# ArthurBrussee/brush

Hardware: AMD Instinct MI355X
Metric: train views/sec @ 1M Gaussians, 1080p (fwd + L1/SSIM loss + bwd + Adam per view) (higher is better)
Workload: dtype f32

## Files before the change

### brush_amd/_ffi.py

```python
import ctypes as C
import os

_DIR = os.path.dirname(os.path.abspath(__file__))
LIB_PATH = os.environ.get("BRUSH_HIP_LIB") or os.path.join(_DIR, "libbrush_hip.so")

FLAG_MIP = 1
FLAG_BWD_INFO = 2
FLAG_SMOOTH_CUTOFF = 4
FLAG_SLICED_LISTS = 8

fp = C.POINTER(C.c_float)
u32p = C.POINTER(C.c_uint32)


class BhCamera(C.Structure):
    _fields_ = [
        ("vm", C.c_float * 12),
        ("fx", C.c_float), ("fy", C.c_float), ("cx", C.c_float), ("cy", C.c_float),
        ("lim_pos_x", C.c_float), ("lim_pos_y", C.c_float),
        ("lim_neg_x", C.c_float), ("lim_neg_y", C.c_float),
        ("cam_pos", C.c_float * 3),
        ("img_w", C.c_uint32), ("img_h", C.c_uint32),
        ("tile_row_begin", C.c_uint32), ("tile_row_end", C.c_uint32),
        ("model", C.c_uint32), ("dist", C.c_float * 8), ("half_max_render_fov", C.c_float),
# ... 440 lines not shown

ABI_VERSION = 7
STRUCT_MIRRORS = (BhCamera, BhRenderOut, BhLossConfig, BhTrainConfig, BhTrainState, BhTrainBatch, BhTrainStats, BhRefineConfig, BhRefineStats, BhPlyInfo)

_lib = None
_lib_th = None
TEST_HOOKS_LIB_PATH = os.path.join(_DIR, "libbrush_hip_testhooks.so")
TEST_HOOK_SYMBOLS = {"bh_debug_fill_train_scratch": (C.c_int, [C.c_void_p, C.c_uint32]),
                     "bh_debug_split_counts": (C.c_int, [C.c_void_p, C.POINTER(C.c_uint32)]),
                     "bh_debug_depth_sort": (C.c_int, [C.c_void_p, C.c_void_p, C.c_void_p, C.c_void_p, C.c_uint32, C.c_void_p, C.c_void_p, C.c_void_p, C.c_void_p,
                                                       C.POINTER(C.c_int), C.POINTER(C.c_uint32)]),
                     "bh_debug_depth_deal": (C.c_int, [C.c_void_p, C.c_void_p, C.c_void_p, C.c_void_p, C.c_uint32, C.c_void_p, C.c_void_p, C.c_void_p, C.c_void_p,
                                                       C.c_uint32, C.c_uint32, C.POINTER(C.c_uint64), C.POINTER(C.c_int)]),
                     "bh_debug_dsort_deal_counts": (C.c_int, [C.c_void_p, C.POINTER(C.c_uint32)]),
                     "bh_debug_set_deal_capacity": (C.c_int, [C.c_void_p, C.c_uint32]),
                     "bh_debug_image_loss_window": (C.c_int, [C.c_void_p, C.c_void_p, C.c_void_p, C.c_uint32, C.c_uint32, C.POINTER(BhLossConfig), C.c_float, C.c_uint32,
                                                              C.c_uint32, C.c_void_p, C.c_void_p])}


class BrushHipError(RuntimeError):
    pass


def _bind(path, symbols):
    if not os.path.exists(path):
        raise BrushHipError(
            "%s not found: build it with `python -c 'import __graft_entry__ as g; g.build()'` "
            "(hipcc --offload-arch=gfx950). There is no CPU fallback." % path)
    lib = C.CDLL(path)
    for name, (res, args) in symbols.items():
# ... 25 lines not shown
```

### brush_amd/csrc/api.hip

```cpp
#include <cmath>
#include <cstdlib>
#include <cstdio>
#include <algorithm>
#include <cstring>
#include <new>

#include "../../include/brush_hip_intrinsics.h"
#include "context.h"
#include "depth_deal.h"
#include "device_rng.h"
#include "param_table.h"

namespace bh {

__global__ __launch_bounds__(256) void zero_two_kernel(float4* __restrict__ a, size_t na, float4* __restrict__ b, size_t nb) {
    const size_t stride = (size_t)gridDim.x * 256;
    const float4 z = make_float4(0.0f, 0.0f, 0.0f, 0.0f);
    for (size_t i = (size_t)blockIdx.x * 256 + threadIdx.x; i < na + nb; i += stride) {
        if (i < na) a[i] = z;
        else b[i - na] = z;
    }
}

int set_error(bh_ctx* ctx, int code, const std::string& msg) {
// ... 301 lines not shown
}
bool parse_flag(const char* v, bool* out) {
    uint32_t x = 0;
    if (!parse_u32(v, 0, 1, &x)) return false;
    *out = x != 0;
    return true;
}
struct Option { const char* name; const char* help; bool (*apply)(bh_ctx* c, const char* v); };
const Option kOptions[] = {
    {"cut_min_pairs", "u32: a view whose last frame had fewer pairs keeps complete lists (= bh_set_list_cut_threshold)",
     [](bh_ctx* c, const char* v) { return parse_u32(v, 0, 0xFFFFFFFFu, &c->cut_min_pairs); }},
    {"cut_margin_pct", "0..10000: base margin behind a tile's last useful splat, % of its depth rank (default 150)",
     [](bh_ctx* c, const char* v) { return parse_u32(v, 0, 10000, &c->knob_cut_margin_pct); }},
    {"cut_margin_fixed", "0|1: the margin is cut_margin_pct for every frame instead of adaptive",
     [](bh_ctx* c, const char* v) { return parse_flag(v, &c->knob_fixed_margin); }},
    {"cut_ctrl", "up:down:floor:gap_exp — the margin controller's constants (default 1.5:0.998:0.5:0.3333)", [](bh_ctx* c, const char* v) {
        float a = 0, b = 0, d = 0, e = 0;
        if (sscanf(v, "%f:%f:%f:%f", &a, &b, &d, &e) != 4 || !(a >= 1.0f && b > 0.0f && b <= 1.0f && d > 0.0f && e >= 0.0f && e <= 1.0f)) return false;
        c->ctrl_up = a; c->ctrl_down = b; c->ctrl_floor = d; c->ctrl_gap_exp = e;
        return true;
    }},
    {"cut_sort_all", "0|1: with per-tile cuts, still depth-sort every visible splat",
     [](bh_ctx* c, const char* v) { return parse_flag(v, &c->knob_cut_sort_all); }},
    {"auto_exact_share", "0..1: a view whose last cut frame listed more than this share of its pairs renders complete lists (default 0.9; 0 = never)", [](bh_ctx* c, const char* v) {
        char* end = nullptr;
        const float x = strtof(v, &end);
        if (end == v || *end != '\0' || !(x >= 0.0f && x <= 1.0f)) return false;
        c->auto_exact_share = x;
        return true;
    }},
    {"no_view_hash", "0|1: frames without a view id share ONE table instead of being keyed by their camera",
     [](bh_ctx* c, const char* v) { return parse_flag(v, &c->knob_no_view_hash); }},
    {"k16_order", "0 index order | 1 by the view's last per-tile work | 2 dealt: the forward blend's tile order",
     [](bh_ctx* c, const char* v) { return parse_u32(v, 0, 2, &c->knob_k16_order); }},
// ... 262 lines not shown
    const float* transforms = req.transforms;
    const float* sh_coeffs = req.sh_coeffs;
    const float* raw_opacities = req.raw_opacities;
    ctx->have_forward = false;
    ctx->clears.begin_forward();
    const bool mip = flags & BH_FLAG_MIP;
    Frame f;
    f.bwd_info = flags & BH_FLAG_BWD_INFO; f.smooth = flags & BH_FLAG_SMOOTH_CUTOFF;
    f.bg[0] = req.bg[0]; f.bg[1] = req.bg[1]; f.bg[2] = req.bg[2];
    f.u = make_uniforms(req.cam);
    if (f.u.tile_y0 >= f.u.tile_y1 || f.u.tile_y1 > f.u.tile_bh) return set_error(ctx, BH_ERR_INVALID_ARG, "tile_row window must satisfy begin < end <= ceil(img_h / 16)");
    f.num_tiles = f.u.tile_bw * f.u.tile_bh;
    const size_t npad = n ? n : 1;

    constexpr size_t counter_set_bytes = COUNTER_SET_BYTES, counter_set_words = COUNTER_SET_BYTES / 4, counter_read_bytes = COUNTER_READ_BYTES;
    auto* counter_pairs = (uint32_t*)ensure(ctx, SLOT_COUNTERS, 2 * counter_set_bytes + 64);
    uint32_t* dev_sums = counter_pairs ? counter_pairs + 2 * counter_set_words : nullptr;
    uint32_t* counters = counter_pairs ? counter_pairs + counter_set_words * (ctx->counter_phase & 1u) : nullptr;
    auto* depth_keys = (uint32_t*)ensure(ctx, SLOT_DEPTH_KEYS, npad * 4);
    auto* isect_counts = (uint32_t*)ensure(ctx, SLOT_ISECT_COUNTS, npad * 4);
    auto* max_radius = req.max_radius ? req.max_radius : (float*)ensure(ctx, SLOT_MAX_RADIUS, npad * 4);
    f.proj_by_gid = (float*)ensure(ctx, SLOT_PROJECTED_BY_GID, npad * 9 * 4);
    if (!counters || !depth_keys || !isect_counts || !max_radius || !f.proj_by_gid) return BH_ERR_OOM;

    f.gfc = (uint32_t*)ensure(ctx, SLOT_GLOBAL_FROM_COMPACT, npad * 4);
    auto* depths_sorted = (uint32_t*)ensure(ctx, SLOT_DEPTHS_SORTED, npad * 4);
    if (!f.gfc || !depths_sorted) return BH_ERR_OOM;
    const bool bwd_jobs = f.bwd_info && ctx->knob_bwd_jobs && !ctx->knob_no_lpt && !((flags & BH_FLAG_SLICED_LISTS) && ctx->slice_fraction > 0.0f);
    const size_t lpt_words = LPT_HEADER_WORDS + (size_t)8 * LPT_CLASSES * band_slots(f.num_tiles);
    auto* tile_offsets = (uint32_t*)ensure(ctx, SLOT_TILE_OFFSETS, ((size_t)f.num_tiles * 2 + lpt_words) * 4);
    f.visible = (f.bwd_info && req.visible) ? req.visible : (float*)ensure(ctx, SLOT_VISIBLE, (f.bwd_info ? npad : 1) * 4);
// ... 33 lines not shown
    bool k5_queued = false;
    uint32_t spec_pair_cap = 0;
    float* spec_projected = nullptr;
    float4* spec_vc = nullptr;
    uint32_t *spec_tile_ids = nullptr, *spec_isect_gids = nullptr;
    if (n > 0) {
        fused_scan = depth_sort_supported(n) && !ctx->knob_generic_depth_sort;
        const bool sums_on_device = fused_scan && !ctx->knob_readback_copy;
        bool* spl_written = nullptr;
        uint32_t* spl_listed = nullptr;
        uint32_t* spl = view_splitters(view, cut_active, &spl_written, &spl_listed);
        if (!spl && ctx->dsort_spl) { spl = ctx->dsort_spl; spl_written = &ctx->dsort_spl_written; spl_listed = &ctx->dsort_spl_keys; }
        DealArgs dealt;
        {
            ProfScope ps(ctx, "ProjectSplats");
            if (!ctx->counters_ready) BH_HIP(ctx, hipMemsetAsync(counter_pairs, 0, 2 * counter_set_bytes, ctx->stream));
            ctx->counters_ready = false;
            ForwardPrep prep;
            prep.next_counters = reinterpret_cast<unsigned long long*>(counter_pairs + counter_set_words * ((ctx->counter_phase & 1u) ^ 1u));
            prep.visible = visible_words ? reinterpret_cast<uint32_t*>(f.visible) : nullptr;
            prep.visible_words = (uint32_t)visible_words;
            prep.tile_table = tile_offsets;
            prep.tile_words = f.num_tiles * 2 + LPT_HEADER_WORDS;
            prep.slice_table = slice_tab;
            prep.slice_words = (uint32_t)slice_words;
            prep.list_all_visible = ctx->knob_cut_sort_all;
            if (view && ctx->knob_k16_order && n >= 8u * 256u) {
                const uint32_t win_t = f.u.tile_bw * (f.u.tile_y1 - f.u.tile_y0);
                tile_order = (uint32_t*)ensure(ctx, SLOT_TILE_ORDER, ((size_t)8 * band_slots(win_t) + SPLIT_TAIL_WORDS) * 4);
                if (!tile_order) return BH_ERR_OOM;
                prep.order_work = vtab + (size_t)f.num_tiles;
// ... 48 lines not shown
                spec_projected = (float*)ensure(ctx, SLOT_PROJECTED, npad * 9 * 4);
                spec_vc = f.bwd_info ? (float4*)ensure(ctx, SLOT_V_COMBINED, npad * 10 * 4 + 16) : nullptr;
                if (!spec_projected || (f.bwd_info && !spec_vc)) return BH_ERR_OOM;
                spec_tile_ids = (uint32_t*)ctx->slots[SLOT_TILE_IDS].ptr;
                spec_isect_gids = (uint32_t*)ctx->slots[SLOT_ISECT_GIDS].ptr;
                spec_pair_cap = (uint32_t)std::min<size_t>(cap_pairs, 0xFFFFFFFEull);
                ProfScope ps(ctx, "MapGaussiansToIntersect");
                BH_TRY(launch_map_gaussians(ctx, n, f.u, f.proj_by_gid, f.gfc, spec_projected, cum_early, spec_tile_ids, spec_isect_gids, spec_vc,
                                            spec_vc ? (uint32_t)(((size_t)n * 10 + 3) / 4) : 0u, 0xFFFFFFFFu, cut_active ? slice_tab : nullptr,
                                            cut_active ? vtab : nullptr, cut_active ? depths_sorted : nullptr, dev_sums + (cut_active ? 3 : 0), spec_pair_cap));
                k5_queued = true;
            }
        }
        if (poll_tag) BH_TRY(wait_host_tag(ctx, reinterpret_cast<const volatile uint32_t*>(hslots) + HOST_SUM_WORDS - 1u, ctx->readback_tag, "count readback"));
        else BH_HIP(ctx, hipEventSynchronize(ctx->readback_ev));
        if (ctx->gate_learn) {
            ctx->gate_learn = false;
            ctx->far_direct = reinterpret_cast<const volatile uint32_t*>(ctx->host_counters)[HOST_GATE_WORD] != 0u;
        }
        unsigned long long hc[4] = {0ull, 0ull, 0ull, 0ull};
        if (sums_on_device) {
            const volatile unsigned long long* hs = hslots;
            for (uint32_t c = 0; c < COUNTER_K1_U64; ++c) hc[c] = hs[c];
        } else {
            for (uint32_t k = 0; k < COUNTER_SLOTS; ++k)
                for (uint32_t c = 0; c < COUNTER_K1_U64; ++c) hc[c] += hslots[COUNTER_K1_U64 * k + c];
        }
        if (hc[1] > 0xFFFFFFFFull) return set_error(ctx, BH_ERR_UNSUPPORTED, "more than 2^32-1 tile intersections");
        nv_true = (uint32_t)hc[0];
        f.ni = (uint32_t)hc[1];
// ... 38 lines not shown
    if (bwd_jobs) {
        const uint32_t listed = cut_active ? near_total : f.ni;
        const uint32_t ckpt_cap = (uint32_t)std::min<uint64_t>((uint64_t)listed / BWD_SEG + f.num_tiles + 1u, BWD_CKPT_MAX_SLOTS);
        f.rs.jobs.ckpt = (float4*)ensure(ctx, SLOT_BWD_CKPT, (size_t)ckpt_cap * 256 * sizeof(float4));
        f.rs.jobs.ckpt_cap = ckpt_cap;
        f.rs.jobs.top_cap = band_slots(f.num_tiles) + ckpt_cap;
        f.rs.jobs.top_list = (uint32_t*)ensure(ctx, SLOT_BWD_TOPLIST, (size_t)8 * f.rs.jobs.top_cap * 4);
        if (!f.rs.jobs.ckpt || !f.rs.jobs.top_list) return BH_ERR_OOM;
    }
    if (view) {
        f.rs.zcut = vtab;
        f.rs.depth_keys_sorted = depths_sorted;
        f.rs.nv = f.nv;
        f.rs.cut_active = by_cut;
        f.rs.margin_pct = cut_margin_pct(ctx, view);
        f.rs.work = vtab + (size_t)f.num_tiles;
        f.rs.order = tile_order;
        f.rs.order_mode = ctx->knob_k16_order;
        f.rs.split = tile_split;
#ifdef BH_TEST_HOOKS
        ctx->last_split = tile_split;
#endif
    }
    const uint32_t win_tiles = f.u.tile_bw * (f.u.tile_y1 - f.u.tile_y0);
    const float class_width_raw = (float)f.ni / (float)(win_tiles ? win_tiles : 1u) / 64.0f;
    f.class_width = ctx->knob_lpt_linear ? (class_width_raw < 8.0f ? 8.0f : class_width_raw) : 0.0f;
    f.lpt = (f.bwd_info && !ctx->knob_no_lpt) ? tile_offsets + (size_t)f.num_tiles * 2 : nullptr;
    f.out_f32 = f.bwd_info ? (float*)out_img : nullptr;
    f.out_u8 = f.bwd_info ? nullptr : (uint32_t*)out_img;

// ... 117 lines not shown
    r.intersect_counts = isect_counts;
    r.depths_sorted = (float*)depths_sorted;
    r.tile_offsets_far = sliced ? f.tile_offsets_far : nullptr;
    r.list_budget = f.budget;
    r.generation = ++ctx->generation;
    ctx->clears.stamp(r.generation);
    *out = r;
    ForwardState& latest = ctx->latest;
    latest.out = r;
    latest.uniforms = f.u;
    latest.n = n; latest.sh_degree = sh_degree; latest.flags = flags;
    latest.bg[0] = f.bg[0]; latest.bg[1] = f.bg[1]; latest.bg[2] = f.bg[2];
    latest.lpt = f.lpt;
    latest.jobs = f.rs.jobs;
    ctx->have_forward = true;
    if (view) view_rendered(view, f.ni);
    return 0;
}

extern "C" {

int bh_set_list_slicing(bh_ctx* ctx, float near_share) {
    if (!ctx) return BH_ERR_INVALID_ARG;
    if (near_share != near_share || near_share > 1.0f) return set_error(ctx, BH_ERR_INVALID_ARG, "set_list_slicing: the near slice's share must be <= 1 (<= 0: automatic)");
    ctx->slice_fraction = near_share > 0.0f ? near_share : 0.0f;
    return 0;
}

int bh_set_list_cut_threshold(bh_ctx* ctx, uint32_t min_pairs) {
    if (!ctx) return BH_ERR_INVALID_ARG;
    ctx->cut_min_pairs = min_pairs;
// ... 8 lines not shown

int bh_forget_views(bh_ctx* ctx) {
    if (!ctx) return BH_ERR_INVALID_ARG;
    BH_HIP(ctx, hipSetDevice(ctx->device));
    if (ctx->far_job.pending) BH_TRY(finish_far_slice(ctx, nullptr));
    if (ctx->dsort_spl) { BH_HIP(ctx, hipMemsetAsync(ctx->dsort_spl, 0, DSORT_SPL_STRIDE * 4, ctx->stream)); ctx->dsort_spl_written = false; ctx->dsort_spl_keys = 0u; }
    if (ctx->views.empty()) return 0;
    BH_HIP(ctx, hipStreamSynchronize(ctx->stream));
    deliver_pending_loss(ctx);
    for (auto& kv : ctx->views)
        if (kv.second.zcut) (void)hipFree(kv.second.zcut);
    ctx->views.clear();
    ctx->casual_views = 0;
    for (uint64_t& k : ctx->seen_keys) k = 0ull;
    ctx->far_job.view = nullptr;
    ctx->margin_scale = 1.0f;
    return 0;
}

float bh_last_list_share(bh_ctx* ctx) { return ctx ? ctx->last_slice_share : 0.0f; }
uint32_t bh_far_slices_queued(bh_ctx* ctx) { return ctx ? ctx->far_launches : 0u; }
uint32_t bh_view_table_count(bh_ctx* ctx) { return ctx ? (uint32_t)ctx->views.size() : 0u; }

}

namespace bh {

int backward_impl(bh_ctx* ctx, const ForwardState& fs, const float* v_output, const BackwardCall& call) {
    const float *transforms = call.transforms, *sh_coeffs = call.sh_coeffs, *raw_opacities = call.raw_opacities;
    float *v_transforms = call.v_transforms, *v_sh_coeffs = call.v_sh_coeffs, *v_raw_opacities = call.v_raw_opacities, *v_refine_weight = call.v_refine_weight;
    const size_t span_floats = call.span_floats;
// ... 390 lines not shown
            ctx->deal_fallbacks++;
            rc = depth_sort_scan(ctx, keys, minmax, counts, n, out_keys, out_vals, cum, nullptr, nullptr, nullptr, 0u, nullptr, spl, &written);
            if (rc == 0) rc = check_hip(ctx, hipStreamSynchronize(ctx->stream), "debug_depth_deal: sync");
        }
    } else {
        (void)hipStreamSynchronize(ctx->stream);
    }
    (void)hipFree(d.ctr);
    return rc;
}
extern "C" int bh_debug_set_deal_capacity(bh_ctx* ctx, uint32_t cap) {
    if (!ctx) return BH_ERR_INVALID_ARG;
    ctx->deal_cap_override = cap;
    return 0;
}
extern "C" int bh_debug_dsort_deal_counts(bh_ctx* ctx, uint32_t* out) {
    if (!ctx || !out) return BH_ERR_INVALID_ARG;
    out[0] = ctx->deal_frames;
    out[1] = ctx->deal_fallbacks;
    return 0;
}
extern "C" int bh_debug_image_loss_window(bh_ctx* ctx, const float* img_hwc4, const uint32_t* gt_packed, uint32_t h, uint32_t w, const BhLossConfig* cfg,
                                          float alpha_weight, uint32_t tile_y0, uint32_t tile_y1, float* loss_out, float* v_output) {
    if (!ctx) return BH_ERR_INVALID_ARG;
    if (!img_hwc4 || !gt_packed || !cfg || !loss_out || !v_output || h == 0 || w == 0)
        return set_error(ctx, BH_ERR_INVALID_ARG, "debug_image_loss_window: bad argument");
    if (tile_y0 >= tile_y1) return set_error(ctx, BH_ERR_INVALID_ARG, "debug_image_loss_window: empty tile-row window");
    BH_HIP(ctx, hipSetDevice(ctx->device));
    const size_t hw = (size_t)h * w;
    const bool alpha = alpha_weight > 0.0f;
// ... 7 lines not shown
```

### brush_amd/csrc/context.h

```cpp
#pragma once
#include <hip/hip_runtime.h>
#include <stdint.h>

#include <memory>
#include <string>
#include <unordered_map>
#include <vector>

#include "../../include/brush_hip.h"
#include "../../include/brush_hip_lpips.h"
#include "../../include/brush_hip_image.h"
#include "../../include/brush_hip_exposure.h"
#include "../../include/brush_hip_bilagrid.h"
#include "../../include/brush_hip_depth_loss.h"
#include "../../include/brush_hip_normal_loss.h"
#include "../../include/brush_hip_distortion.h"
#include "../../include/brush_hip_mesh.h"
#include "../../include/brush_hip_features.h"
#include "../../include/brush_hip_feature_train.h"
#include "../../include/brush_hip_envmap.h"
#include "device_math.h"

namespace bh {

enum Slot : int {
    SLOT_COUNTERS = 0,
    SLOT_DEPTH_KEYS,
    SLOT_ISECT_COUNTS,
    SLOT_MAX_RADIUS,
    SLOT_SORT_KEYS_A,
    SLOT_SORT_KEYS_B,
    SLOT_SORT_VALS_A,
    SLOT_SORT_VALS_B,
    SLOT_SORT_HIST,
    SLOT_COMM_SCRATCH,
// ... 72 lines not shown
};

constexpr int MAX_PROF = 32;

constexpr uint32_t COUNTER_SLOTS = 128;
constexpr uint32_t COUNTER_K1_U64 = 4;
constexpr size_t COUNTER_SET_BYTES = COUNTER_SLOTS * 8 * COUNTER_K1_U64 + COUNTER_SLOTS * 8;
constexpr uint32_t COUNTER_SET_U64 = (uint32_t)(COUNTER_SET_BYTES / 8);
constexpr uint32_t COUNTER_MINMAX_WORD = COUNTER_SLOTS * 2 * COUNTER_K1_U64;
constexpr uint32_t SLICE_CTRL_WORDS = 8;
constexpr uint32_t SORT_GROUP_BLOCKS = 32;
constexpr uint32_t FAR_GROUP_BLOCKS = 64;
constexpr size_t COUNTER_READ_BYTES = COUNTER_SLOTS * 8 * COUNTER_K1_U64;
constexpr uint32_t HOST_SUM_WORDS = 2 * COUNTER_K1_U64 + 1;
constexpr uint32_t HOST_DEAL_WORD = HOST_SUM_WORDS;
constexpr size_t HOST_LOSS_WORD = 16 + COUNTER_READ_BYTES / 4;
constexpr size_t HOST_GATE_WORD = HOST_LOSS_WORD + 16;
constexpr size_t HOST_GATE_TAG_WORD = HOST_GATE_WORD + 1;
constexpr size_t HOST_COUNTERS_BYTES = 64 + COUNTER_READ_BYTES + 64 + 64;

struct Profiler {
    int level = 0;
    const char* names[MAX_PROF];
    float ms[MAX_PROF];
    uint32_t calls[MAX_PROF];
    int count = 0;
    struct Pending { int idx; hipEvent_t a, b; };
    std::vector<Pending> pending;
    std::vector<hipEvent_t> pool;
    hipEvent_t ext_a = nullptr, ext_b = nullptr;
};

constexpr uint32_t ZCUT_ALL = 0xFFFFFFFEu;
BH_DEV bool zcut_near(uint32_t key, uint32_t cut) { return (key >> 1) <= (cut >> 1); }
struct ViewState {
    uint32_t* zcut = nullptr;
    uint32_t tile_bw = 0, tile_bh = 0;
    bool seeded = false;
    uint32_t exact_frames = 0;
    uint32_t penalty = 0;
    uint64_t last_used = 0;
    uint32_t gap = 0;
    uint32_t last_pairs = 0;
    uint32_t complete_frames = 0;
    bool spl_written[2] = {false, false};
    uint32_t spl_keys[2] = {0, 0};
    bool casual = false;
};
constexpr uint32_t CUT_MIN_PAIRS = 1500000u;
constexpr uint32_t LPT_CLASSES = 64;
constexpr uint32_t LPT_HEADER_WORDS = 8 * LPT_CLASSES + 64;
constexpr uint32_t BWD_SEG = 128;
constexpr uint32_t BWD_MAX_SEGS = 64;
struct BwdJobs {
    float4* ckpt = nullptr;
    uint32_t ckpt_cap = 0;
    uint32_t* top_list = nullptr;
    uint32_t top_cap = 0;
// ... 38 lines not shown
    uint32_t* done_bits = nullptr;
    uint32_t* unsat_count = nullptr;
    uint32_t* gate_host = nullptr;
    float* state = nullptr;
    const uint32_t* offsets_near = nullptr;
    uint32_t* zcut = nullptr;
    const uint32_t* depth_keys_sorted = nullptr;
    uint32_t nv = 0;
    bool cut_active = false;
    uint32_t* live_bands = nullptr;
    uint32_t* work = nullptr;
    const uint32_t* order = nullptr;
    uint32_t order_mode = 1;
    uint32_t* split = nullptr;
    uint32_t margin_pct = 150;
    BwdJobs jobs{};
};

struct ForwardRequest {
    BhCamera cam{};
    uint32_t n = 0, sh_degree = 0, flags = 0;
    const float* transforms = nullptr;
    const float* sh_coeffs = nullptr;
    const float* raw_opacities = nullptr;
    float bg[3] = {0, 0, 0};
    uint32_t view_id = 0;
    float* visible = nullptr;
    float* max_radius = nullptr;
    size_t visible_floats = 0;
    float* grad_begin = nullptr;
// ... 174 lines not shown
    int comm_rank = 0, comm_world = 1;
    float slice_fraction = 0.0f;
    float last_slice_share = 1.0f;
    bool far_direct = false;
    uint32_t readback_tag = 0;
    uint32_t gate_tag = 0;
    bool gate_signal_queued = false;
    bool gate_learn = false;
    uint32_t far_launches = 0;
    std::unordered_map<uint64_t, bh::ViewState> views;
    uint64_t seen_keys[bh::SEEN_KEYS] = {};
    uint32_t seen_pos = 0;
    uint32_t casual_views = 0;
    uint32_t view_id = 0;
    uint64_t view_clock = 0;
    float margin_scale = 1.0f;
    float ctrl_up = 1.5f, ctrl_down = 0.998f, ctrl_floor = 0.5f, ctrl_gap_exp = 1.0f / 3.0f;
    uint32_t cut_min_pairs = bh::CUT_MIN_PAIRS;
    bool knob_spec_k5 = true;
    bool knob_event_waits = false;
    bool knob_readback_copy = false;
    bool knob_no_view_hash = false;
    bool knob_fixed_margin = false;
    bool knob_cut_sort_all = false;
    uint32_t feature_chunk = 0;
    uint32_t knob_band_mode = 1;
    uint32_t knob_k16_waves = 0;
    uint32_t knob_k16_split = 250;
    uint32_t knob_k16_split_min = bh::SPLIT_MIN_WORK;
    uint32_t knob_k16_split_of_max = 45;
    const uint32_t* last_split = nullptr;
    uint32_t knob_k16_order = 1;
// ... 84 lines not shown
int launch_bilagrid_slice(bh_ctx* ctx, const bh_bilagrid* tab, uint32_t view, const float* img, uint32_t h, uint32_t w, float* out);
int launch_bilagrid_backward(bh_ctx* ctx, bh_bilagrid* tab, uint32_t view, const float* img, const float* v_sliced, uint32_t h, uint32_t w, float* v_img,
                             float tv_weight, bool update);
int launch_bilagrid_tv(bh_ctx* ctx, const bh_bilagrid* tab, uint32_t view, float* value, float weight, float* accum, float* accum_host);
float* bilagrid_tv_scratch(bh_ctx* ctx);
int check_envmap_frame(bh_ctx* ctx, const BhCamera* cam, uint32_t h, uint32_t w, const char* who);
int launch_envmap_composite(bh_ctx* ctx, const bh_envmap* map, const BhCamera& cam, const float* img, uint32_t h, uint32_t w, float* out);
int launch_envmap_backward(bh_ctx* ctx, bh_envmap* map, const BhCamera& cam, const float* img, const float* v_out, uint32_t h, uint32_t w, float* v_img,
                           bool update, float gscale, bool check_host);
int launch_envmap_adam(bh_ctx* ctx, bh_envmap* map, float gscale);
ViewState* frame_view(bh_ctx* ctx, const ForwardRequest& req, uint32_t tile_bw, uint32_t tile_bh, bool casual);
bool cut_this_frame(const bh_ctx* ctx, ViewState* vs, bool allow_cut);
uint32_t* view_table(const ViewState* vs);
uint32_t* view_splitters(ViewState* vs, bool cut, bool** written, uint32_t** listed = nullptr);
uint32_t cut_margin_pct(const bh_ctx* ctx, const ViewState* vs);
uint32_t list_budget(bh_ctx* ctx, ViewState* cut_view, uint32_t near_total, uint32_t ni);
void view_rendered(ViewState* vs, uint32_t ni);
int enqueue_far_slice(bh_ctx* ctx, const FarJob& j);
int finish_far_slice(bh_ctx* ctx, bool* launched);
bool far_job_decides_first(const bh_ctx* ctx);
void drop_far_job(bh_ctx* ctx);
inline void deliver_pending_loss(bh_ctx* ctx) {
    if (ctx->pending_loss_dst) {
        *ctx->pending_loss_dst = reinterpret_cast<const volatile float*>(ctx->host_counters)[HOST_LOSS_WORD];
        ctx->pending_loss_dst = nullptr;
    }
}
int check_hip(bh_ctx* ctx, hipError_t e, const char* what);
int lpips_train_term(bh_ctx* ctx, const float* img_hwc4, const uint32_t* gt_packed, uint32_t h, uint32_t w, const float* bg, float* v_output,
                     float* loss, float* loss_host);
std::string ply_header_comments(uint32_t sh_degree, bool render_mip, const float* up_axis);
enum ResizeOut : int { RESIZE_OUT_U8 = 0, RESIZE_OUT_PACKED = 1, RESIZE_OUT_PACKED_PREMUL = 2 };
// ... 163 lines not shown
```

### brush_amd/csrc/depth_sort.hip

```cpp
#include <cstddef>

#include "context.h"
#include "depth_deal.h"
#include "sort_groups.h"

namespace bh {

constexpr int DS_WG = 256;
constexpr int DS_WAVES = DS_WG / 64;
#define BH_DS_KPT 8
constexpr int DS_KPT = BH_DS_KPT;
constexpr int DS_TILE = DS_WG * DS_KPT;
constexpr int DS_RADIX = 256;
constexpr uint32_t CULLED_KEY = 0xFFFFFFFFu;

struct DepthSplit {
    uint32_t kmin, kmax;
    uint32_t scale;
    bool any_visible;
    const uint32_t* spl;
};
constexpr uint32_t SPL_WORDS = 258;
static_assert(SPL_WORDS <= DSORT_SPL_STRIDE, "context.h reserves the table");
constexpr uint32_t SPL_MIN_KEYS = 16384;
// ... 79 lines not shown
    }
#pragma unroll
    for (int off = 32; off > 0; off >>= 1) {
#pragma unroll
        for (uint32_t c = 0; c < COUNTER_K1_U64; ++c) tot[c] += __shfl_down(tot[c], off);
    }
    if (lane == 0) {
        if (dev_sums) {
#pragma unroll
            for (uint32_t c = 0; c < COUNTER_K1_U64; ++c) dev_sums[c] = deal_overflow ? 0u : (tot[c] > 0xFFFFFFFFull ? 0xFFFFFFFFu : (uint32_t)tot[c]);
        }
        volatile unsigned long long* h64 = reinterpret_cast<volatile unsigned long long*>(host_sums);
#pragma unroll
        for (uint32_t c = 0; c < COUNTER_K1_U64; ++c) h64[c] = tot[c];
        reinterpret_cast<volatile uint32_t*>(host_sums)[HOST_DEAL_WORD] = deal_overflow;
        if (tag) {
            __threadfence_system();
            reinterpret_cast<volatile uint32_t*>(host_sums)[HOST_SUM_WORDS - 1u] = tag;
        }
    }
}

__global__ __launch_bounds__(DS_WG) void dsort_hist_kernel(const uint32_t* __restrict__ keys, const uint32_t* __restrict__ counts,
                                                          uint32_t n, uint32_t nblocks, const uint32_t* __restrict__ minmax,
                                                          uint32_t* __restrict__ hist , SortGroups grp, uint32_t ngroups,
                                                          const uint32_t* __restrict__ rb_set, uint32_t* __restrict__ rb_host, uint32_t rb_tag, uint32_t* __restrict__ rb_dev,
                                                          const uint32_t* __restrict__ spl_in, uint8_t* __restrict__ digits ) {
    __shared__ uint32_t s_hist[DS_WAVES][DS_RADIX];
    __shared__ uint32_t s_csum[DS_WAVES][DS_RADIX];
    __shared__ uint32_t s_red[2 * DS_WAVES];
// ... 711 lines not shown
```

### brush_amd/csrc/lists.hip

```cpp
#include <algorithm>
#include <cmath>
#include <cstring>

#include "context.h"

namespace bh {

static uint64_t view_key(const bh_ctx* ctx, uint32_t view_id, const BhCamera& c) {
    if (view_id != 0u || ctx->knob_no_view_hash) return (uint64_t)view_id;
    uint64_t h = 0x9E3779B97F4A7C15ull;
    auto mix = [&](uint32_t w) {
        h += (uint64_t)w + 0x9E3779B97F4A7C15ull;
        uint64_t z = h;
        z = (z ^ (z >> 30)) * 0xBF58476D1CE4E5B9ull;
        z = (z ^ (z >> 27)) * 0x94D049BB133111EBull;
        h = z ^ (z >> 31);
    };
    auto bits = [](float f) { uint32_t u; std::memcpy(&u, &f, 4); return u; };
    for (int i = 0; i < 12; ++i) mix(bits(c.vm[i]));
    mix(bits(c.fx)); mix(bits(c.fy)); mix(bits(c.cx)); mix(bits(c.cy));
    mix(c.img_w); mix(c.img_h); mix(c.tile_row_begin); mix(c.tile_row_end); mix(c.model);
    if (c.model != BH_CAMERA_PINHOLE) for (int i = 0; i < 8; ++i) mix(bits(c.dist[i]));
    return h | (1ull << 63);
}
// ... 83 lines not shown
        vs->complete_frames--;
    } else if (vs->exact_frames) {
        vs->exact_frames--;
    }
    return false;
}

uint32_t* view_table(const ViewState* vs) { return vs ? vs->zcut : nullptr; }

uint32_t* view_splitters(ViewState* vs, bool cut, bool** written, uint32_t** listed) {
    *written = vs ? &vs->spl_written[cut ? 1 : 0] : nullptr;
    if (listed) *listed = vs ? &vs->spl_keys[cut ? 1 : 0] : nullptr;
    return vs ? vs->zcut + 2 * (size_t)vs->tile_bw * vs->tile_bh + (cut ? DSORT_SPL_STRIDE : 0u) : nullptr;
}

uint32_t cut_margin_pct(const bh_ctx* ctx, const ViewState* vs) {
    if (ctx->knob_fixed_margin) return ctx->knob_cut_margin_pct;
    const float gap = vs && vs->gap > 2u ? (float)vs->gap : 2.0f;
    const float m = (float)ctx->knob_cut_margin_pct * ctx->margin_scale * std::pow(gap * 0.5f, ctx->ctrl_gap_exp);
    return m < 6400.0f ? (m > 10.0f ? (uint32_t)m : 10u) : 6400u;
}

uint32_t list_budget(bh_ctx* ctx, ViewState* cut_view, uint32_t near_total, uint32_t ni) {
    uint32_t budget = ni;
    const float share = ctx->slice_fraction;
    if (share > 0.0f) {
        if (share < 1.0f) {
            const double b = (double)share * (double)ni;
            const uint32_t floor_b = ni < 1024u ? ni : 1024u;
            budget = b < (double)floor_b ? floor_b : (uint32_t)b;
            if (budget > ni) budget = ni;
        }
        ctx->last_slice_share = (float)((double)budget / (double)ni);
    } else if (cut_view && near_total < ni) {
        budget = near_total;
        const float cut_share = (float)((double)near_total / (double)ni);
        ctx->last_slice_share = cut_share;
        if (ctx->auto_exact_share > 0.0f && cut_share > ctx->auto_exact_share) cut_view->complete_frames = AUTO_EXACT_FRAMES;
    } else {
        if (cut_view && ctx->auto_exact_share > 0.0f) cut_view->complete_frames = AUTO_EXACT_FRAMES;
        ctx->last_slice_share = 1.0f;
    }
    return budget;
}

void view_rendered(ViewState* vs, uint32_t ni) {
    vs->seeded = true;
    vs->last_pairs = ni;
}

static void view_outcome(bh_ctx* ctx, ViewState* vs, bool missed, bool shared_table) {
    if (!ctx->knob_fixed_margin) {
        const float s = ctx->margin_scale * (missed ? ctx->ctrl_up : ctx->ctrl_down);
        ctx->margin_scale = s < ctx->ctrl_floor ? ctx->ctrl_floor : (s > 16.0f ? 16.0f : s);
    }
    if (!vs) return;
    vs->penalty = ((vs->penalty << 1) | (missed ? 1u : 0u)) & 0xFFu;
    if (__builtin_popcount(vs->penalty) >= (shared_table ? 3 : 6)) {
        vs->exact_frames = shared_table ? 32u : 8u;
        vs->penalty = 0u;
    }
}

int enqueue_far_slice(bh_ctx* ctx, const FarJob& j) {
    const Frame& f = j.frame;
    const uint32_t* gate = f.slice_info + 2;
    const uint32_t far_max = f.ni;
    {
        ProfScope ps(ctx, "MapGaussiansToIntersect");
// ... 66 lines not shown
```

### brush_amd/csrc/rasterize.hip

```cpp
#include <hip/hip_ext.h>

#include <type_traits>

#include "context.h"
#include "device_blend.h"

namespace bh {

struct OffsetsDyn {
    const uint32_t* n_dev = nullptr;
    const uint32_t* gate = nullptr;
    const uint32_t* base = nullptr;
};
__global__ __launch_bounds__(256) void tile_offsets_kernel(const uint32_t* __restrict__ tile_ids, uint32_t num_isect,
                                                          uint32_t num_tiles, uint32_t* __restrict__ tile_offsets, OffsetsDyn dyn) {
    uint32_t ofs = 0;
    if (dyn.gate && *dyn.gate == 0u) return;
    if (dyn.n_dev) { const uint32_t v = *dyn.n_dev; num_isect = v < num_isect ? v : num_isect; }
    if (dyn.base) { ofs = *dyn.base; tile_ids += ofs; }
    const uint32_t i0 = (blockIdx.x * 256 + threadIdx.x) * 4u;
    if (i0 >= num_isect) return;
    uint32_t t[4];
    if (i0 + 4u <= num_isect && (ofs & 3u) == 0u) {
        const uint4 v = *reinterpret_cast<const uint4*>(&tile_ids[i0]);
// ... 89 lines not shown


struct SliceArgs {
    uint32_t* done_bits = nullptr;
    uint32_t* unsat_count = nullptr;
    uint32_t* gate_host = nullptr;
    float* state = nullptr;
    const uint32_t* offsets_near = nullptr;
    uint32_t* zcut = nullptr;
    const uint32_t* depth_keys_sorted = nullptr;
    uint32_t nv = 0;
    uint32_t cut_active = 0;
    uint32_t* live_bands = nullptr;
    uint32_t tile_bh = 0;
    uint32_t margin_pct = 150;
    const uint32_t* order = nullptr;
    uint32_t order_mode = 1;
    uint32_t* split = nullptr;
    uint32_t* work = nullptr;
    BwdJobs jobs{};
};

template <bool BWD_INFO, bool SMOOTH, int PHASE, int NQ>
BH_DEV void blend_tile(const RasterUniforms& u, const uint32_t* __restrict__ isect_gids, uint32_t* __restrict__ tile_offsets,
                       const float* __restrict__ projected, const uint32_t* __restrict__ global_from_compact, float* __restrict__ out_img,
                       uint32_t* __restrict__ out_packed, float* __restrict__ visible, uint32_t* __restrict__ lpt, const SliceArgs& sl,
                       float* s_splat, const uint32_t local_tile, const uint32_t qsel, uint32_t* split_row) {
    constexpr int NK = NQ == 4 ? 2 : 1;
    const uint32_t bidx = blockIdx.x;
    const uint32_t tile = u.tile_begin + local_tile;
// ... 327 lines not shown
            const uint32_t cls = size >= BWD_SEG ? LPT_CLASSES - 1u : (size * (LPT_CLASSES - 1u)) / BWD_SEG;
            const uint32_t band = bidx & 7u;
            const uint32_t pos = atomicAdd(&lpt[band * LPT_CLASSES + cls], 1u);
            const uint32_t entry = local_tile | ((uint32_t)lane << JOB_SEG_SHIFT) | (last ? JOB_LAST_BIT : 0u);
            if (cls == LPT_CLASSES - 1u) sl.jobs.top_list[(size_t)band * sl.jobs.top_cap + pos] = entry;
            else lpt[lpt_list_offset(u.num_tiles, band, cls) + pos] = entry;
        }
    }
    if (lane == 0) {
        if (PHASE == 1) atomicOr(&sl.done_bits[tile >> 5], 1u << (tile & 31u));
        uint32_t work = (BWD_INFO ? last_useful : reached) - range_lo;
        if (PHASE == 2) {
            const uint32_t n_lo = sl.offsets_near[tile * 2], n_hi = sl.offsets_near[tile * 2 + 1];
            work += n_hi - n_lo;
        }
        if (sl.work) sl.work[tile] = work;
        if (BWD_INFO) {
            tile_offsets[tile * 2 + 1] = last_useful;
            if (lpt && !sl.jobs.ckpt) {
                uint32_t cls;
                if (u.rcp_class_width > 0.0f) {
                    cls = min(LPT_CLASSES - 1u, (uint32_t)((float)work * u.rcp_class_width));
                } else if (work < 8u) {
                    cls = 0u;
                } else {
                    const uint32_t p = 28u - (uint32_t)__builtin_clz(work);
                    cls = min(LPT_CLASSES - 1u, 1u + 8u * p + ((work >> p) & 7u));
                }
                const uint32_t list = (bidx & 7u) * LPT_CLASSES + cls;
                const uint32_t pos = atomicAdd(&lpt[list], 1u);
                lpt[lpt_list_offset(u.num_tiles, bidx & 7u, cls) + pos] = local_tile | JOB_LAST_BIT;
// ... 80 lines not shown
    u.bg_r = bg[0]; u.bg_g = bg[1]; u.bg_b = bg[2];
    SliceArgs sl;
    if (slice) {
        sl.done_bits = slice->done_bits;
        sl.unsat_count = slice->unsat_count;
        sl.gate_host = phase == 1 ? slice->gate_host : nullptr;
        sl.state = slice->state;
        sl.offsets_near = slice->offsets_near;
        sl.zcut = slice->zcut;
        sl.depth_keys_sorted = slice->depth_keys_sorted;
        sl.nv = slice->nv;
        sl.cut_active = slice->cut_active ? 1u : 0u;
        sl.live_bands = slice->live_bands;
        sl.tile_bh = vu.tile_bh;
        sl.margin_pct = slice->margin_pct;
        sl.order = slice->order;
        sl.order_mode = slice->order_mode;
        sl.split = (phase != 2 && slice->order && slice->order_mode == 1u) ? slice->split : nullptr;
        sl.work = slice->work;
        if (bwd_info && phase != 2 && lpt) sl.jobs = slice->jobs;
    }
    if (sl.zcut && (!sl.depth_keys_sorted && sl.nv)) sl.zcut = nullptr;
    if (phase != 0 && (!sl.done_bits || !sl.unsat_count || !sl.state || (phase == 2 && !sl.offsets_near)))
        return set_error(ctx, BH_ERR_INVALID_ARG, "launch_rasterize: sliced phase without its scratch");
    uint32_t nblocks = band_slots(u.num_tiles) * 8u;
    if (sl.order && sl.order_mode == 2u) nblocks = ((band_slots(u.num_tiles) + 7u) / 8u) * 64u;
    if (sl.split) nblocks += 8u * 3u * SPLIT_MAX;
    const dim3 grid(nblocks);
    uint32_t lds_pad = 0;
    if (ctx->knob_k16_waves >= 1u && ctx->knob_k16_waves < 8u && sl.order && sl.order_mode == 1u && phase != 2) {
// ... 280 lines not shown
```

Before: 1336.

## Drive cut margin controller from device-reported per-tile work growth

Replaces the purely miss/hit multiplicative margin scale with a policy that also tracks the maximum per-tile work growth that saturated tiles report from the rasterizer via atomics, read back alongside the existing count readback. The margin is set to the larger of the held scale and safety times the decayed tracked growth, and misses caused by a heavy tail below a near threshold no longer inflate the scale. The aim is to keep per-tile depth cuts tight enough to skip far splats while avoiding repeated misses that force complete re-renders. It adds a few atomics in the blend kernel's epilogue and extra state in the host controller.

```diff
diff --git a/brush_amd/_ffi.py b/brush_amd/_ffi.py
--- a/brush_amd/_ffi.py
+++ b/brush_amd/_ffi.py
@@ -478,6 +478,7 @@
                                                        C.c_uint32, C.c_uint32, C.POINTER(C.c_uint64), C.POINTER(C.c_int)]),
                      "bh_debug_dsort_deal_counts": (C.c_int, [C.c_void_p, C.POINTER(C.c_uint32)]),
                      "bh_debug_set_deal_capacity": (C.c_int, [C.c_void_p, C.c_uint32]),
+                     "bh_debug_cut_report": (C.c_int, [C.c_void_p, C.c_uint32, C.POINTER(C.c_uint32), C.c_void_p, C.c_uint32]),
                      "bh_debug_image_loss_window": (C.c_int, [C.c_void_p, C.c_void_p, C.c_void_p, C.c_uint32, C.c_uint32, C.POINTER(BhLossConfig), C.c_float, C.c_uint32,
                                                               C.c_uint32, C.c_void_p, C.c_void_p])}
 
diff --git a/brush_amd/csrc/api.hip b/brush_amd/csrc/api.hip
--- a/brush_amd/csrc/api.hip
+++ b/brush_amd/csrc/api.hip
@@ -339,10 +339,16 @@
      [](bh_ctx* c, const char* v) { return parse_u32(v, 0, 10000, &c->knob_cut_margin_pct); }},
     {"cut_margin_fixed", "0|1: the margin is cut_margin_pct for every frame instead of adaptive",
      [](bh_ctx* c, const char* v) { return parse_flag(v, &c->knob_fixed_margin); }},
-    {"cut_ctrl", "up:down:floor:gap_exp — the margin controller's constants (default 1.5:0.998:0.5:0.3333)", [](bh_ctx* c, const char* v) {
-        float a = 0, b = 0, d = 0, e = 0;
-        if (sscanf(v, "%f:%f:%f:%f", &a, &b, &d, &e) != 4 || !(a >= 1.0f && b > 0.0f && b <= 1.0f && d > 0.0f && e >= 0.0f && e <= 1.0f)) return false;
+    {"cut_ctrl", "up:down:floor:gap_exp[:safety:decay:near] — the margin controller's constants (default 1.5:0.998:0.5:0.3333:1.5:0.98:0.5): the margin is x up after a miss, x down "
+                 "after a hit, never below floor x cut_margin_pct, x (gap / 2)^gap_exp for a view that comes back after gap frames; it tracks safety x the decayed (x decay per cut "
+                 "frame that held) maximum of the growth the cut frames' tiles report; a miss whose reporters stayed below near x the margin leaves it alone (safety x near <= 1)",
+     [](bh_ctx* c, const char* v) {
+        float a = 0, b = 0, d = 0, e = 0, s = c->ctrl_safety, y = c->ctrl_decay, r = c->ctrl_near;
+        const int got = sscanf(v, "%f:%f:%f:%f:%f:%f:%f", &a, &b, &d, &e, &s, &y, &r);
+        if ((got != 4 && got != 7) || !(a >= 1.0f && b > 0.0f && b <= 1.0f && d > 0.0f && e >= 0.0f && e <= 1.0f)) return false;
+        if (!(s >= 1.0f && s <= 16.0f && y > 0.0f && y <= 1.0f && r >= 0.0f && s * r <= 1.0f)) return false;
         c->ctrl_up = a; c->ctrl_down = b; c->ctrl_floor = d; c->ctrl_gap_exp = e;
+        c->ctrl_safety = s; c->ctrl_decay = y; c->ctrl_near = r;
         return true;
     }},
     {"cut_sort_all", "0|1: with per-tile cuts, still depth-sort every visible splat",
@@ -635,7 +641,7 @@
     const size_t npad = n ? n : 1;
 
     constexpr size_t counter_set_bytes = COUNTER_SET_BYTES, counter_set_words = COUNTER_SET_BYTES / 4, counter_read_bytes = COUNTER_READ_BYTES;
-    auto* counter_pairs = (uint32_t*)ensure(ctx, SLOT_COUNTERS, 2 * counter_set_bytes + 64);
+    auto* counter_pairs = (uint32_t*)ensure(ctx, SLOT_COUNTERS, 2 * counter_set_bytes + DEV_SUMS_WORDS * 4);
     uint32_t* dev_sums = counter_pairs ? counter_pairs + 2 * counter_set_words : nullptr;
     uint32_t* counters = counter_pairs ? counter_pairs + counter_set_words * (ctx->counter_phase & 1u) : nullptr;
     auto* depth_keys = (uint32_t*)ensure(ctx, SLOT_DEPTH_KEYS, npad * 4);
@@ -699,7 +705,7 @@
         DealArgs dealt;
         {
             ProfScope ps(ctx, "ProjectSplats");
-            if (!ctx->counters_ready) BH_HIP(ctx, hipMemsetAsync(counter_pairs, 0, 2 * counter_set_bytes, ctx->stream));
+            if (!ctx->counters_ready) BH_HIP(ctx, hipMemsetAsync(counter_pairs, 0, 2 * counter_set_bytes + DEV_SUMS_WORDS * 4, ctx->stream));
             ctx->counters_ready = false;
             ForwardPrep prep;
             prep.next_counters = reinterpret_cast<unsigned long long*>(counter_pairs + counter_set_words * ((ctx->counter_phase & 1u) ^ 1u));
@@ -778,6 +784,7 @@
         }
         if (poll_tag) BH_TRY(wait_host_tag(ctx, reinterpret_cast<const volatile uint32_t*>(hslots) + HOST_SUM_WORDS - 1u, ctx->readback_tag, "count readback"));
         else BH_HIP(ctx, hipEventSynchronize(ctx->readback_ev));
+        cut_report_arrived(ctx, sums_on_device ? reinterpret_cast<const volatile uint32_t*>(hslots) + HOST_REPORT_WORD : nullptr);
         if (ctx->gate_learn) {
             ctx->gate_learn = false;
             ctx->far_direct = reinterpret_cast<const volatile uint32_t*>(ctx->host_counters)[HOST_GATE_WORD] != 0u;
@@ -846,6 +853,11 @@
         f.rs.nv = f.nv;
         f.rs.cut_active = by_cut;
         f.rs.margin_pct = cut_margin_pct(ctx, view);
+        if (by_cut) {
+            f.rs.report = fused_scan && !ctx->knob_generic_depth_sort && !ctx->knob_readback_copy ? dev_sums + DEV_REPORT_MAX_WORD : nullptr;
+            f.rs.report_pct = view->margin_written;
+            cut_report_armed(ctx, view);
+        }
         f.rs.work = vtab + (size_t)f.num_tiles;
         f.rs.order = tile_order;
         f.rs.order_mode = ctx->knob_k16_order;
@@ -993,7 +1005,7 @@
     latest.lpt = f.lpt;
     latest.jobs = f.rs.jobs;
     ctx->have_forward = true;
-    if (view) view_rendered(view, f.ni);
+    if (view) view_rendered(view, f.ni, f.rs.margin_pct);
     return 0;
 }
 
@@ -1032,7 +1044,8 @@
     ctx->casual_views = 0;
     for (uint64_t& k : ctx->seen_keys) k = 0ull;
     ctx->far_job.view = nullptr;
-    ctx->margin_scale = 1.0f;
+    ctx->cut_state = CutState{};
+    ctx->cut_report = bh_ctx::CutReport{};
     return 0;
 }
 
@@ -1453,6 +1466,26 @@
     ctx->deal_cap_override = cap;
     return 0;
 }
+extern "C" int bh_debug_cut_report(bh_ctx* ctx, uint32_t view_id, uint32_t* out, uint32_t* table, uint32_t tiles) {
+    if (!ctx || !out) return BH_ERR_INVALID_ARG;
+    BH_HIP(ctx, hipSetDevice(ctx->device));
+    BH_HIP(ctx, hipStreamSynchronize(ctx->stream));
+    out[0] = out[1] = 0u;
+    const uint32_t* counter_pairs = (const uint32_t*)ctx->slots[SLOT_COUNTERS].ptr;
+    if (counter_pairs) {
+        const uint32_t* dev_sums = counter_pairs + 2 * (COUNTER_SET_BYTES / 4);
+        BH_HIP(ctx, hipMemcpy(&out[0], dev_sums + DEV_REPORT_MAX_WORD, 4, hipMemcpyDeviceToHost));
+        BH_HIP(ctx, hipMemcpy(&out[1], dev_sums + DEV_REPORT_COUNT_WORD, 4, hipMemcpyDeviceToHost));
+    }
+    out[2] = cut_margin_pct(ctx, nullptr);
+    out[3] = ctx->cut_report.armed ? 1u : 0u;
+    if (table) {
+        auto it = ctx->views.find((uint64_t)view_id);
+        if (it == ctx->views.end() || (size_t)it->second.tile_bw * it->second.tile_bh != tiles) return -1;
+        BH_HIP(ctx, hipMemcpy(table, it->second.zcut, (size_t)tiles * 2 * 4, hipMemcpyDeviceToHost));
+    }
+    return 0;
+}
 extern "C" int bh_debug_dsort_deal_counts(bh_ctx* ctx, uint32_t* out) {
     if (!ctx || !out) return BH_ERR_INVALID_ARG;
     out[0] = ctx->deal_frames;
diff --git a/brush_amd/csrc/context.h b/brush_amd/csrc/context.h
--- a/brush_amd/csrc/context.h
+++ b/brush_amd/csrc/context.h
@@ -19,6 +19,7 @@
 #include "../../include/brush_hip_features.h"
 #include "../../include/brush_hip_feature_train.h"
 #include "../../include/brush_hip_envmap.h"
+#include "cut_policy.h"
 #include "device_math.h"
 
 namespace bh {
@@ -121,6 +122,9 @@
 constexpr size_t COUNTER_READ_BYTES = COUNTER_SLOTS * 8 * COUNTER_K1_U64;
 constexpr uint32_t HOST_SUM_WORDS = 2 * COUNTER_K1_U64 + 1;
 constexpr uint32_t HOST_DEAL_WORD = HOST_SUM_WORDS;
+constexpr uint32_t HOST_REPORT_WORD = HOST_DEAL_WORD + 1;
+constexpr uint32_t DEV_SUMS_WORDS = 128;
+constexpr uint32_t DEV_REPORT_MAX_WORD = 32, DEV_REPORT_COUNT_WORD = 64;
 constexpr size_t HOST_LOSS_WORD = 16 + COUNTER_READ_BYTES / 4;
 constexpr size_t HOST_GATE_WORD = HOST_LOSS_WORD + 16;
 constexpr size_t HOST_GATE_TAG_WORD = HOST_GATE_WORD + 1;
@@ -149,6 +153,7 @@
     uint64_t last_used = 0;
     uint32_t gap = 0;
     uint32_t last_pairs = 0;
+    uint32_t margin_written = 0;
     uint32_t complete_frames = 0;
     bool spl_written[2] = {false, false};
     uint32_t spl_keys[2] = {0, 0};
@@ -217,6 +222,8 @@
     uint32_t order_mode = 1;
     uint32_t* split = nullptr;
     uint32_t margin_pct = 150;
+    uint32_t* report = nullptr;
+    uint32_t report_pct = 0;
     BwdJobs jobs{};
 };
 
@@ -421,8 +428,15 @@
     uint32_t casual_views = 0;
     uint32_t view_id = 0;
     uint64_t view_clock = 0;
-    float margin_scale = 1.0f;
+    bh::CutState cut_state;
     float ctrl_up = 1.5f, ctrl_down = 0.998f, ctrl_floor = 0.5f, ctrl_gap_exp = 1.0f / 3.0f;
+    float ctrl_safety = 1.5f, ctrl_decay = 0.98f, ctrl_near = 0.5f;
+    struct CutReport {
+        bool armed = false;
+        bool outcome = false;
+        bool missed = false;
+        float margin_pct = 0.0f, gap = 2.0f;
+    } cut_report;
     uint32_t cut_min_pairs = bh::CUT_MIN_PAIRS;
     bool knob_spec_k5 = true;
     bool knob_event_waits = false;
@@ -537,8 +551,10 @@
 uint32_t* view_table(const ViewState* vs);
 uint32_t* view_splitters(ViewState* vs, bool cut, bool** written, uint32_t** listed = nullptr);
 uint32_t cut_margin_pct(const bh_ctx* ctx, const ViewState* vs);
+void cut_report_armed(bh_ctx* ctx, const ViewState* vs);
+void cut_report_arrived(bh_ctx* ctx, const volatile uint32_t* words);
 uint32_t list_budget(bh_ctx* ctx, ViewState* cut_view, uint32_t near_total, uint32_t ni);
-void view_rendered(ViewState* vs, uint32_t ni);
+void view_rendered(ViewState* vs, uint32_t ni, uint32_t margin_pct);
 int enqueue_far_slice(bh_ctx* ctx, const FarJob& j);
 int finish_far_slice(bh_ctx* ctx, bool* launched);
 bool far_job_decides_first(const bh_ctx* ctx);
diff --git a/brush_amd/csrc/cut_policy.h b/brush_amd/csrc/cut_policy.h
--- /dev/null
+++ b/brush_amd/csrc/cut_policy.h
@@ -0,0 +1,59 @@
+#pragma once
+#include <cmath>
+#include <cstdint>
+
+namespace bh {
+
+constexpr uint32_t CUT_GROWTH_ONE = 1u << 16;
+constexpr uint32_t CUT_REPORT_UNKNOWN = 0xFFFFFFFFu;
+constexpr uint32_t CUT_REPORT_MIN_WORK = 32;
+constexpr float CUT_MARGIN_MIN_PCT = 10.0f, CUT_MARGIN_MAX_PCT = 6400.0f;
+constexpr float CUT_SCALE_MAX = 16.0f;
+
+struct CutCtrl {
+    float base_pct;
+    float up, down;
+    float floor;
+    float gap_exp;
+    float safety;
+    float decay;
+    float near;
+};
+struct CutState {
+    float scale = 1.0f;
+    float growth = 0.0f;
+};
+struct CutFrame {
+    bool missed;
+    uint32_t growth_fx;
+    uint32_t reporters;
+    float margin_pct;
+    float gap;
+};
+
+inline float cut_gap_factor(const CutCtrl& c, float gap) { return std::pow((gap > 2.0f ? gap : 2.0f) * 0.5f, c.gap_exp); }
+
+inline uint32_t cut_policy_margin(const CutCtrl& c, const CutState& s, float gap) {
+    const float held = c.base_pct * s.scale, tracked = 100.0f * c.safety * s.growth;
+    const float m = (held > tracked ? held : tracked) * cut_gap_factor(c, gap);
+    return m < CUT_MARGIN_MAX_PCT ? (m > CUT_MARGIN_MIN_PCT ? (uint32_t)m : (uint32_t)CUT_MARGIN_MIN_PCT) : (uint32_t)CUT_MARGIN_MAX_PCT;
+}
+
+inline bool cut_heavy_tail(const CutCtrl& c, const CutFrame& f) {
+    return f.missed && f.reporters != CUT_REPORT_UNKNOWN && (float)f.growth_fx * (100.0f / (float)CUT_GROWTH_ONE) < c.near * f.margin_pct;
+}
+
+inline CutState cut_policy_next(const CutCtrl& c, CutState s, const CutFrame& f) {
+    if (!f.missed) s.growth *= c.decay;
+    if (f.reporters != CUT_REPORT_UNKNOWN && f.reporters != 0u) {
+        float g = (float)f.growth_fx / (float)CUT_GROWTH_ONE / cut_gap_factor(c, f.gap);
+        const float g_max = CUT_MARGIN_MAX_PCT * 0.01f / (c.safety > 0.0f ? c.safety : 1.0f);
+        g = g < g_max ? g : g_max;
+        if (g > s.growth) s.growth = g;
+    }
+    if (!cut_heavy_tail(c, f)) s.scale *= f.missed ? c.up : c.down;
+    s.scale = s.scale < c.floor ? c.floor : (s.scale > CUT_SCALE_MAX ? CUT_SCALE_MAX : s.scale);
+    return s;
+}
+
+}
diff --git a/brush_amd/csrc/depth_sort.hip b/brush_amd/csrc/depth_sort.hip
--- a/brush_amd/csrc/depth_sort.hip
+++ b/brush_amd/csrc/depth_sort.hip
@@ -117,6 +117,12 @@
 #pragma unroll
         for (uint32_t c = 0; c < COUNTER_K1_U64; ++c) h64[c] = tot[c];
         reinterpret_cast<volatile uint32_t*>(host_sums)[HOST_DEAL_WORD] = deal_overflow;
+        if (dev_sums) {
+            reinterpret_cast<volatile uint32_t*>(host_sums)[HOST_REPORT_WORD] = dev_sums[DEV_REPORT_MAX_WORD];
+            reinterpret_cast<volatile uint32_t*>(host_sums)[HOST_REPORT_WORD + 1u] = dev_sums[DEV_REPORT_COUNT_WORD];
+            dev_sums[DEV_REPORT_MAX_WORD] = 0u;
+            dev_sums[DEV_REPORT_COUNT_WORD] = 0u;
+        }
         if (tag) {
             __threadfence_system();
             reinterpret_cast<volatile uint32_t*>(host_sums)[HOST_SUM_WORDS - 1u] = tag;
diff --git a/brush_amd/csrc/lists.hip b/brush_amd/csrc/lists.hip
--- a/brush_amd/csrc/lists.hip
+++ b/brush_amd/csrc/lists.hip
@@ -121,11 +121,33 @@
     return vs ? vs->zcut + 2 * (size_t)vs->tile_bw * vs->tile_bh + (cut ? DSORT_SPL_STRIDE : 0u) : nullptr;
 }
 
+static CutCtrl cut_ctrl(const bh_ctx* ctx) {
+    return CutCtrl{(float)ctx->knob_cut_margin_pct, ctx->ctrl_up, ctx->ctrl_down, ctx->ctrl_floor, ctx->ctrl_gap_exp, ctx->ctrl_safety, ctx->ctrl_decay, ctx->ctrl_near};
+}
+
 uint32_t cut_margin_pct(const bh_ctx* ctx, const ViewState* vs) {
     if (ctx->knob_fixed_margin) return ctx->knob_cut_margin_pct;
-    const float gap = vs && vs->gap > 2u ? (float)vs->gap : 2.0f;
-    const float m = (float)ctx->knob_cut_margin_pct * ctx->margin_scale * std::pow(gap * 0.5f, ctx->ctrl_gap_exp);
-    return m < 6400.0f ? (m > 10.0f ? (uint32_t)m : 10u) : 6400u;
+    return cut_policy_margin(cut_ctrl(ctx), ctx->cut_state, vs ? (float)vs->gap : 2.0f);
+}
+
+void cut_report_armed(bh_ctx* ctx, const ViewState* vs) {
+    ctx->cut_report = bh_ctx::CutReport{};
+    ctx->cut_report.armed = true;
+    ctx->cut_report.margin_pct = (float)vs->margin_written;
+    ctx->cut_report.gap = (float)vs->gap;
+}
+
+void cut_report_arrived(bh_ctx* ctx, const volatile uint32_t* words) {
+    const bh_ctx::CutReport r = ctx->cut_report;
+    ctx->cut_report = bh_ctx::CutReport{};
+    if (!r.armed || !r.outcome || ctx->knob_fixed_margin) return;
+    CutFrame f;
+    f.missed = r.missed;
+    f.growth_fx = words ? words[0] : 0u;
+    f.reporters = words ? words[1] : CUT_REPORT_UNKNOWN;
+    f.margin_pct = r.margin_pct;
+    f.gap = r.gap;
+    ctx->cut_state = cut_policy_next(cut_ctrl(ctx), ctx->cut_state, f);
 }
 
 uint32_t list_budget(bh_ctx* ctx, ViewState* cut_view, uint32_t near_total, uint32_t ni) {
@@ -151,15 +173,16 @@
     return budget;
 }
 
-void view_rendered(ViewState* vs, uint32_t ni) {
+void view_rendered(ViewState* vs, uint32_t ni, uint32_t margin_pct) {
     vs->seeded = true;
     vs->last_pairs = ni;
+    vs->margin_written = margin_pct;
 }
 
 static void view_outcome(bh_ctx* ctx, ViewState* vs, bool missed, bool shared_table) {
-    if (!ctx->knob_fixed_margin) {
-        const float s = ctx->margin_scale * (missed ? ctx->ctrl_up : ctx->ctrl_down);
-        ctx->margin_scale = s < ctx->ctrl_floor ? ctx->ctrl_floor : (s > 16.0f ? 16.0f : s);
+    if (ctx->cut_report.armed) {
+        ctx->cut_report.outcome = true;
+        ctx->cut_report.missed = missed;
     }
     if (!vs) return;
     vs->penalty = ((vs->penalty << 1) | (missed ? 1u : 0u)) & 0xFFu;
diff --git a/brush_amd/csrc/rasterize.hip b/brush_amd/csrc/rasterize.hip
--- a/brush_amd/csrc/rasterize.hip
+++ b/brush_amd/csrc/rasterize.hip
@@ -127,6 +127,8 @@
     uint32_t* live_bands = nullptr;
     uint32_t tile_bh = 0;
     uint32_t margin_pct = 150;
+    uint32_t* report = nullptr;
+    uint32_t report_pct = 0;
     const uint32_t* order = nullptr;
     uint32_t order_mode = 1;
     uint32_t* split = nullptr;
@@ -484,7 +486,20 @@
             const uint32_t n_lo = sl.offsets_near[tile * 2], n_hi = sl.offsets_near[tile * 2 + 1];
             work += n_hi - n_lo;
         }
-        if (sl.work) sl.work[tile] = work;
+        if (sl.work) {
+            if (sl.report && saturated) {
+                const uint32_t before = sl.work[tile];
+                if (before >= CUT_REPORT_MIN_WORK && work > before) {
+                    const unsigned long long grown = work - before;
+                    if (grown * 400ull > (unsigned long long)before * sl.report_pct) {
+                        const unsigned long long fx = grown * CUT_GROWTH_ONE / before;
+                        atomicMax(&sl.report[0], fx < 0xFFFFFFFFull ? (uint32_t)fx : 0xFFFFFFFFu);
+                        atomicAdd(&sl.report[DEV_REPORT_COUNT_WORD - DEV_REPORT_MAX_WORD], 1u);
+                    }
+                }
+            }
+            sl.work[tile] = work;
+        }
         if (BWD_INFO) {
             tile_offsets[tile * 2 + 1] = last_useful;
             if (lpt && !sl.jobs.ckpt) {
@@ -595,6 +610,8 @@
         sl.live_bands = slice->live_bands;
         sl.tile_bh = vu.tile_bh;
         sl.margin_pct = slice->margin_pct;
+        sl.report = slice->report;
+        sl.report_pct = slice->report_pct;
         sl.order = slice->order;
         sl.order_mode = slice->order_mode;
         sl.split = (phase != 2 && slice->order && slice->order_mode == 1u) ? slice->split : nullptr;
```

After: 1334. No clear change (-0.2%).
